# whwh747/A-Low-Texture-Robust-Hybrid-Feature-Based-Visual-Odometry

Measured on AMD Instinct MI355X. Metric: RGB-D frames/sec (640×480, 1k ORB + LSD + PEAC) at 1/2/4/8 GPUs, higher is better.
Workload: dtype u8/u16 integer + f32/f64; 1 GPU; 640x480 synthetic RGB-D, 1000 ORB (quota; 3/4 std + 1/4 lowtex scenes) + LSD lines + PEAC planes, 8192 frames per GPU per step (std640); frames_per_gpu=8192, parallelism=frames sharded, 1 rank(s), no data-path collective, distinct_frames=256, resident_bytes_per_frame_estimate=21100000

## Files before the change

a-low-texture-robust-hybrid-feature-based-visual-odometry_amd/__init__.py:

```python
import ctypes as C
import os
import subprocess
import numpy as np

_HERE = os.path.dirname(os.path.abspath(__file__))
_CSRC = os.path.join(_HERE, "csrc")
_LIBPATH = os.environ.get("HVO_LIB") or os.path.join(_CSRC, "libhvo.so")
_LIB = None
_LOADED_BEFORE_TORCH = False

HVO_OK = 0
STAGE_ORB, STAGE_LSD, STAGE_PLANES, STAGE_ALL = 1, 2, 4, 7
SLAB_LABELS = 1
STAGE_LSD_CULL = 8
STAGE_LINES3D, STAGE_VP, STAGE_PLANE_TAIL, STAGE_GRIDS = 16, 32, 64, 128
STAGE_FRAME = 1 | 2 | 8 | 4 | 16 | 32 | 64 | 128
LINE_MATCH_NNR, LINE_MATCH_BF, LINE_MATCH_DOUBLE = 0, 1, 2

KEYPOINT_DT = np.dtype([("x", "<f4"), ("y", "<f4"), ("size", "<f4"), ("angle", "<f4"),
                        ("response", "<f4"), ("octave", "<i4"), ("class_id", "<i4")])
KEYLINE_DT = np.dtype([("angle", "<f4"), ("class_id", "<i4"), ("octave", "<i4"),
                       ("pt_x", "<f4"), ("pt_y", "<f4"), ("response", "<f4"), ("size", "<f4"),
                       ("sx", "<f4"), ("sy", "<f4"), ("ex", "<f4"), ("ey", "<f4"),
                       ("sox", "<f4"), ("soy", "<f4"), ("eox", "<f4"), ("eoy", "<f4"),
# ... 1123 lines not shown
        self._chk(lib().hvo_normals_lpvo(self.h, _p(depth), w, h, depth.strides[0], _p(nrm), _p(dz), _p(px), cap, C.byref(n)), "normals_lpvo")
        return nrm[: n.value], dz[: n.value], px[: n.value]

    def surface_normals(self, depth):
        depth = np.ascontiguousarray(depth, np.uint16); h, w = depth.shape
        cap = (((h + 2) // 3) // 2) * (((w + 2) // 3) // 2)
        out = np.zeros(max(cap, 1), SURFACE_NORMAL_DT); n = C.c_int(0)
        self._chk(lib().hvo_surface_normals(self.h, _p(depth), w, h, depth.strides[0], _p(out), cap, C.byref(n)), "surface_normals")
        return out[: n.value].copy()

    def lsd_images(self, frame=0):
        L = lib()
        L.hvo_debug_lsd_images.argtypes = [C.c_void_p, C.c_int, C.POINTER(C.c_int), C.POINTER(C.c_int), C.c_void_p, C.c_void_p, C.c_longlong, C.POINTER(C.c_longlong), C.c_void_p]
        L.hvo_debug_lsd_images.restype = C.c_int
        w, h = self._w, self._h
        sw, sh = int(round(w * 0.8)), int(round(h * 0.8))
        mask = np.zeros((sh, (sw + 31) // 32), np.uint32); rec = np.zeros((sw * sh, 4), np.float64); dxy = np.zeros((h, w, 2), np.int16)
        n = C.c_longlong(0); csw = C.c_int(0); csh = C.c_int(0)
        self._chk(L.hvo_debug_lsd_images(self.h, frame, C.byref(csw), C.byref(csh), _p(mask), _p(rec), len(rec), C.byref(n), _p(dxy)), "lsd_images")
        if (csw.value, csh.value) != (sw, sh):
            raise HvoError(-1, "lsd_images: the plan's scaled size is %d x %d" % (csw.value, csh.value))
        return {"mask": mask, "records": rec[:n.value].copy(), "dxy": dxy}

    def peac_stats(self, frame=0):
        L = lib()
        L.hvo_debug_peac_stats.argtypes = [C.c_void_p, C.c_int, C.c_void_p]; L.hvo_debug_peac_stats.restype = C.c_int
        m = np.zeros(16, np.int32)
        self._chk(L.hvo_debug_peac_stats(self.h, frame, _p(m)), "peac_stats")
        return {"segments": int(m[0]), "coarse_planes": int(m[2]), "flags": int(m[3]), "planes": int(m[4]), "queue_entries": int(m[5]),
                "flood_rounds": int(m[8]), "flood_ranked_rounds": int(m[9]), "flood_serial_rounds": int(m[10]), "ahc_rounds": int(m[11]), "ahc_stops_no_head": int(m[12]), "ahc_stops_conflict": int(m[13]), "ahc_stops_key_order": int(m[14])}

    def hamming_matrix(self, q, t):
        q = np.ascontiguousarray(q, np.uint8).reshape(-1, 32); t = np.ascontiguousarray(t, np.uint8).reshape(-1, 32)
        d = np.zeros((len(q), len(t)), np.uint16)
        self._chk(lib().hvo_hamming_matrix(self.h, _p(q), len(q), _p(t), len(t), _p(d)), "hamming_matrix")
        return d

    def hamming_knn2(self, q, t):
        q = np.ascontiguousarray(q, np.uint8).reshape(-1, 32); t = np.ascontiguousarray(t, np.uint8).reshape(-1, 32)
        idx = np.zeros((len(q), 2), np.int32); dist = np.zeros((len(q), 2), np.int32)
        self._chk(lib().hvo_hamming_knn2(self.h, _p(q), len(q), _p(t), len(t), _p(idx), _p(dist)), "hamming_knn2")
        return idx, dist

    def match_nnr(self, d1, d2, nnr):
        d1 = np.ascontiguousarray(d1, np.uint8).reshape(-1, 32); d2 = np.ascontiguousarray(d2, np.uint8).reshape(-1, 32)
        m = np.full(len(d1), -1, np.int32); n = C.c_int(0)
# ... 869 lines not shown
```

a-low-texture-robust-hybrid-feature-based-visual-odometry_amd/csrc/lsd.hip:

```cpp
#include "hvo_internal.hpp"
#include <math.h>
#include <string.h>
#include <vector>
#include <algorithm>

#define LSD_PI 3.1415926535897932384626433832795
#define LSD_NOTDEF (-1024.0)
#ifndef LSD_RING
#define LSD_RING 256
#endif

static double lsd_sqrt_threshold(double rho)
{
    double c = rho * rho;
    while (sqrt(nextafter(c, INFINITY)) <= rho) c = nextafter(c, INFINITY);
    while (sqrt(c) > rho) c = nextafter(c, 0.0);
    return c;
}

struct LsdPlan {
    int w = 0, h = 0, sw = 0, sh = 0, batch = 0, nfeat = 0, nwords = 0;
    double *d_blur = nullptr;
    int chunk = 0;
    double4 *d_px = nullptr;
    bool compact = false; double4 *d_pool = nullptr; size_t pool_cap = 0;
    unsigned *d_defmask = nullptr, *d_wprefix = nullptr;
    long long *d_fbase = nullptr; int *d_fcount = nullptr; unsigned long long *d_pooltop = nullptr;
    unsigned *d_defined = nullptr;
    int *d_reg = nullptr;
    float *d_segs = nullptr;
    hvo_keyline *d_kl_all = nullptr;
    int maxseg = 0;
    hvo_keyline *d_kl = nullptr; uint8_t *d_desc = nullptr; double *d_fn = nullptr; int *d_nkl = nullptr; int *d_flags = nullptr;
    hvo_keyline *d_kl2 = nullptr; uint8_t *d_desc2 = nullptr; double *d_fn2 = nullptr; int *d_nkl2 = nullptr;
    uint8_t *d_b5 = nullptr; short2 *d_dxy = nullptr;
    int *d_xofs = nullptr, *d_yofs = nullptr; float *d_xa = nullptr, *d_yb = nullptr;
    double k7[4] = { 0, 0, 0, 0 };
    int k5[3] = { 0, 0, 0 };
    double gL[21], gG[63];
    float *d_gL = nullptr, *d_gG = nullptr;
    double rho = 0, prec = 0, p = 0; unsigned min_reg = 0;
    double rhoT = 0;
    long long *d_stats = nullptr;
    bool pre_fused = true;
    struct { Knob dense, lat, async_w, async_early, async_lds, lat_lds, lbd_split, spin_max; } kn;
    uint8_t *d_b8 = nullptr, *d_s8 = nullptr; int *d_rs8tab = nullptr;
    size_t async_w_cap = 0;
    int *d_redo = nullptr; int async_last_n = 0, async_last_w = 0;
    int async_b = 0; unsigned *d_atags = nullptr; void *d_actl = nullptr; int *d_alists = nullptr, *d_ablk = nullptr, *d_afreg = nullptr; unsigned char *d_ainreg = nullptr; int ainreg_b = 0;
};
static LsdPlan *plan_of(hvo_ctx *ctx) { return (LsdPlan *)ctx->lsd; }

static __device__ __forceinline__ int refl(int p, int n) { if (p < 0) p = -p; if (p >= n) p = 2 * (n - 1) - p; return p < 0 ? 0 : p; }

static __device__ __forceinline__ float fatan2_deg(float y, float x)
{
    const float p1 = 0.9997878412794807f * (float)(180 / 3.14159265358979323846);
    const float p3 = -0.3258083974640975f * (float)(180 / 3.14159265358979323846);
    const float p5 = 0.1555786518463281f * (float)(180 / 3.14159265358979323846);
    const float p7 = -0.04432655554792128f * (float)(180 / 3.14159265358979323846);
    const float eps = (float)2.2204460492503131e-16;
    const float ax = fabsf(x), ay = fabsf(y);
    const bool hi = ax >= ay;
    const float c = __fdiv_rn(hi ? ay : ax, __fadd_rn(hi ? ax : ay, eps)), c2 = __fmul_rn(c, c);
    float r = __fmul_rn(__fadd_rn(__fmul_rn(__fadd_rn(__fmul_rn(__fadd_rn(__fmul_rn(p7, c2), p5), c2), p3), c2), p1), c);
    if (!hi) r = __fsub_rn(90.f, r);
    if (x < 0) r = __fsub_rn(180.f, r);
    if (y < 0) r = __fsub_rn(360.f, r);
// ... 1021 lines not shown
        rowstep(v + 1, nB, nA);
    }
    if (v == v1) rowstep(v, nA, nB);
    if (yb + LBD_FUSED_ROWS >= h) store_edge(h - 1, nA, nB);
}

template <bool AL>
__global__ __launch_bounds__(256) void k_lbd_blur_sobel(const uint8_t *__restrict__ gray, size_t gframe, int gpitch,
                                                        short2 *__restrict__ dxy, int w, int h, int k0, int k1, int k2)
{
    const int nstrip = (w + 3) >> 2, item = blockIdx.x * 256 + threadIdx.x, f = blockIdx.z;
    const int rb = item / nstrip;
    const int x0 = (item - rb * nstrip) * 4, yb = rb * LBD_FUSED_ROWS;
    if (yb >= h) return;
    lbd_blur_sobel_body<AL>(gray + (size_t)f * gframe, gpitch, dxy + (size_t)f * h * w, w, h, x0, yb, k0, k1, k2);
}

__constant__ int c_lbd_comb[32][2] = {
    { 0, 1 }, { 0, 2 }, { 0, 3 }, { 0, 4 }, { 0, 5 }, { 0, 6 }, { 1, 2 }, { 1, 3 }, { 1, 4 }, { 1, 5 }, { 1, 6 },
    { 2, 3 }, { 2, 4 }, { 2, 5 }, { 2, 6 }, { 2, 7 }, { 2, 8 }, { 3, 4 }, { 3, 5 }, { 3, 6 }, { 3, 7 }, { 3, 8 },
    { 4, 5 }, { 4, 6 }, { 4, 7 }, { 4, 8 }, { 5, 6 }, { 5, 7 }, { 5, 8 }, { 6, 7 }, { 6, 8 }, { 7, 8 } };

#define LBD_UNR 8
__global__ __launch_bounds__(64) void k_lbd_desc(const short2 *__restrict__ dxyImg, int w, int h,
                                                 const hvo_keyline *__restrict__ kls, const int *__restrict__ nkl, int kl_cap,
                                                 const float *__restrict__ gL, const float *__restrict__ gG, uint8_t *__restrict__ desc)
{
    __shared__ float rows[63][4];
    __shared__ float band[9][8];
    __shared__ float dv[72];
    const int line = blockIdx.x, f = blockIdx.y, t = threadIdx.x;
    if (line >= nkl[f]) return;
    const hvo_keyline kl = kls[(size_t)f * kl_cap + line];
    const short2 *DXY = dxyImg + (size_t)f * w * h;
    const short imageWidth = (short)(w - 1), imageHeight = (short)(h - 1);
    const short halfHeight = 31;
    const short lengthOfLSP = (short)kl.num_pixels;
    const short halfWidth = (short)((lengthOfLSP - 1) / 2);
    const float midX = (float)(0.5 * (double)__fadd_rn(kl.sox, kl.eox));
    const float midY = (float)(0.5 * (double)__fadd_rn(kl.soy, kl.eoy));
    const float dL0 = (float)cos((double)kl.angle), dL1 = (float)sin((double)kl.angle);
    const float dO0 = -dL1, dO1 = dL0;
    __shared__ int tile[63 * 33];
    const bool along_rows = fabsf(dL0) > fabsf(dL1);
    float sCorX = 0, sCorY = 0, pL = 0, nL = 0, pO = 0, nO = 0;
    if (t < 63) {
        float sCorX0 = __fadd_rn(__fadd_rn(__fmul_rn(-dL0, (float)halfWidth), __fmul_rn(dL1, (float)halfHeight)), midX);
        float sCorY0 = __fadd_rn(__fsub_rn(__fmul_rn(-dL1, (float)halfWidth), __fmul_rn(dL0, (float)halfHeight)), midY);
        for (int q = 0; q < t; q++) { sCorX0 = __fsub_rn(sCorX0, dL1); sCorY0 = __fadd_rn(sCorY0, dL0); }
// ... 107 lines not shown
        }
        tempM = __fdiv_rn(1.f, sqrtf(tempM)); tempS = __fdiv_rn(1.f, sqrtf(tempS));
        v0 = __fmul_rn(v0, (t & 7) < 4 ? tempM : tempS); v1 = __fmul_rn(v1, (t & 7) < 4 ? tempM : tempS);
        if ((double)v0 > 0.4) v0 = (float)0.4;
        if ((double)v1 > 0.4) v1 = (float)0.4;
        p0 = __fmul_rn(v0, v0); p1 = __fmul_rn(v1, v1);
        float tmp = 0;
#pragma unroll
        for (int i = 0; i < 72; i++) tmp = __fadd_rn(tmp, i < 64 ? lane_of(p0, i & 63) : lane_of(p1, i & 7));
        tmp = __fdiv_rn(1.f, sqrtf(tmp));
        __syncthreads();
        dv[t] = __fmul_rn(v0, tmp);
        if (t < 8) dv[64 + t] = __fmul_rn(v1, tmp);
    }
    __syncthreads();
    if (t < 32) {
        const float *f1 = dv + 8 * c_lbd_comb[t][0], *f2 = dv + 8 * c_lbd_comb[t][1];
        unsigned r = 0;
        for (int b = 0; b < 8; b++) if (f1[b] > f2[b]) r |= 1u << b;
        desc[((size_t)f * kl_cap + line) * 32 + t] = (uint8_t)r;
    }
}


#define CULL_MAXL 2048
struct CullArgs {
    const hvo_keyline *kl; const double *fn; const int *nkl; hvo_keyline *tmp; hvo_keyline *kl_out; double *fn_out; int *nkl_out;
    int cap, tmp_stride, w, h; double dis, cos_th, endpoint_dis;
};

static __device__ double cull_point_line_distance(const float *l, float px, float py)
{
    const double x0 = (double)px, y0 = (double)py, x1 = l[0], y1 = l[1], x2 = l[2], y2 = l[3];
    return fabs((y2 - y1) * x0 + (x1 - x2) * y0 + ((x2 * y1) - (x1 * y2))) / sqrt((y2 - y1) * (y2 - y1) + (x1 - x2) * (x1 - x2));
}
static __device__ double cull_two_line_angle(const double *f1, const double *f2)
{
    double v1[3] = { f1[0], f1[1], f1[2] }, v2[3] = { f2[0], f2[1], f2[2] };
    v1[0] /= v1[2]; v1[1] /= v1[2];
    v2[0] /= v2[2]; v2[1] /= v2[2];
    const double a0 = v1[0] / v1[2], a1 = v1[1] / v1[2], b0 = v2[0] / v2[2], b1 = v2[1] / v2[2];
    const double a = a0 * b0 + a1 * b1;
    const double b = sqrt(a0 * a0 + a1 * a1), c = sqrt(b0 * b0 + b1 * b1);
    return fabs(a / (b * c));
}
static __device__ void cull_merge_two_lines(const float *l1, const float *l2, float *out)
// ... 110 lines not shown
    double *fo = a.fn_out + (size_t)f * a.cap * 3;
    for (int i = lane; i < m; i += 64) {
        const float r = resp[i];
        int rank = 0;
        for (int q = 0; q < m; q++) { const float rq = resp[q]; rank += (rq > r) || (rq == r && q < i); }
        hvo_keyline k = tmp[i]; k.class_id = rank;
        if (rank < a.cap) {
            out[rank] = k;
            const double sx = k.sx, sy = k.sy, ex = k.ex, ey = k.ey;
            const double l0 = sy * 1.0 - 1.0 * ey, l1 = 1.0 * ex - sx * 1.0, l2 = sx * ey - sy * ex;
            const double nrm = sqrt(l0 * l0 + l1 * l1);
            fo[3 * rank] = l0 / nrm; fo[3 * rank + 1] = l1 / nrm; fo[3 * rank + 2] = l2 / nrm;
        }
    }
    if (lane == 0) a.nkl_out[f] = m;
}

void lsd_free(hvo_ctx *ctx)
{
    LsdPlan *P = plan_of(ctx);
    if (!P) return;
    void *ptrs[] = { P->d_kl2, P->d_desc2, P->d_fn2, P->d_nkl2, P->d_blur, P->d_px, P->d_defined, P->d_reg, P->d_segs, P->d_kl_all, P->d_kl,
                     P->d_desc, P->d_fn, P->d_nkl, P->d_flags, P->d_b5, P->d_dxy, P->d_xofs, P->d_yofs, P->d_xa, P->d_yb, P->d_gL, P->d_gG, P->d_stats,
                     P->d_pool, P->d_defmask, P->d_wprefix, P->d_fbase, P->d_fcount, P->d_pooltop, P->d_atags, P->d_actl, P->d_alists, P->d_ablk, P->d_afreg, P->d_ainreg, P->d_redo, P->d_b8, P->d_s8, P->d_rs8tab };
    for (void *q : ptrs) if (q) (void)hipFree(q);
    delete P;
    ctx->lsd = nullptr;
}

static int cvfloor_f(float v) { int i = (int)v; return i - (i > v); }

static int lsd_build_plan(hvo_ctx *ctx, int w, int h, int batch);
static int lsd_ensure_plan(hvo_ctx *ctx, int w, int h, int batch)
{
    LsdPlan *P = plan_of(ctx);
    if (P && P->w == w && P->h == h && P->batch >= batch) return HVO_OK;
    lsd_free(ctx);
    const int rc = lsd_build_plan(ctx, w, h, batch);
    if (rc) lsd_free(ctx);
    return rc;
}

static int lsd_build_plan(hvo_ctx *ctx, int w, int h, int batch)
{
    LsdPlan *P = new LsdPlan();
    ctx->lsd = P;
    P->w = w; P->h = h; P->batch = batch; P->nfeat = std::max(ctx->p.lsd_nfeatures, 1);
// ... 22 lines not shown
        for (int i = 0; i < 21; i++) { double d = i - u; P->gL[i] = exp(d * d * inv); }
        u = (9 * 7 - 1) / 2; sigma = u; inv = -1 / (2 * sigma * sigma);
        for (int i = 0; i < 63; i++) { double d = i - u; P->gG[i] = exp(d * d * inv); }
    }
    std::vector<int> xofs(P->sw), yofs(P->sh + PRE_CH, 0); std::vector<float> xa(2 * P->sw), yb(2 * (P->sh + PRE_CH), 0.f);
    const double scale = 1. / SCALE;
    for (int dx = 0; dx < P->sw; dx++) {
        float fx = (float)((dx + 0.5) * scale - 0.5); int sx = cvfloor_f(fx); fx -= sx;
        if (sx < 0) { fx = 0; sx = 0; }
        if (sx >= w - 1) { fx = 0; sx = w - 1; }
        xofs[dx] = sx; xa[2 * dx] = 1.f - fx; xa[2 * dx + 1] = fx;
    }
    for (int dy = 0; dy < P->sh; dy++) {
        float fy = (float)((dy + 0.5) * scale - 0.5); int sy = cvfloor_f(fy); fy -= sy;
        int sy0 = std::min(std::max(sy, 0), h - 1), sy1 = std::min(std::max(sy + 1, 0), h - 1);
        yofs[dy] = sy0 | (sy1 << 16); yb[2 * dy] = 1.f - fy; yb[2 * dy + 1] = fy;
    }
    std::vector<float> gLf(21), gGf(63);
    for (int i = 0; i < 21; i++) gLf[i] = (float)P->gL[i];
    for (int i = 0; i < 63; i++) gGf[i] = (float)P->gG[i];
    const size_t B = batch, npix = (size_t)w * h, nsp = (size_t)P->sw * P->sh;
#define PA(ptr, n) HVO_HIP(hipMalloc((void **)&(ptr), (n)))
    P->kn.dense.read("HVO_LSD_DENSE"); P->kn.lat.read("HVO_LSD_LAT"); P->kn.async_w.read("HVO_LSD_ASYNC"); P->kn.async_early.read("HVO_LSD_ASYNC_EARLY");
    P->kn.async_lds.read("HVO_LSD_ASYNC_LDS"); P->kn.lat_lds.read("HVO_LSD_LAT_LDS"); P->kn.lbd_split.read("HVO_LBD_SPLIT"); P->kn.spin_max.read("HVO_LSD_ASYNC_SPIN_MAX");
    P->chunk = (int)std::min<size_t>(B, 512);
    { const char *e = getenv("HVO_LSD_CHUNK"); if (e && atoi(e) > 0) P->chunk = (int)std::min<size_t>(B, (size_t)atoi(e)); }
    P->compact = false;
    { const char *e = getenv("HVO_LSD_COMPACT"); if (e) P->compact = atoi(e) != 0; }
    double frac = 0.27;
    { const char *e = getenv("HVO_LSD_COMPACT_FRAC"); if (e && atof(e) > 0) frac = std::min(1.0, atof(e)); }
    if (P->compact) {
        const size_t fit = std::max<size_t>(64, (size_t)(3.3e9 / (double)(nsp * sizeof(double4))) / 64 * 64);
        P->chunk = (int)std::min<size_t>((size_t)P->chunk, std::min<size_t>(fit, 512));
    }
    const size_t CB = (size_t)P->chunk;
    { const char *e = getenv("HVO_LSD_PRE_SPLIT"); P->pre_fused = !(e && atoi(e) != 0); }
    if (!P->pre_fused) PA(P->d_blur, CB * npix * 8);
    if (P->compact) {
        PA(P->d_px, CB * nsp * sizeof(double4));
        P->pool_cap = std::max<size_t>((size_t)((double)(B * nsp) * frac), 4096);
        PA(P->d_pool, P->pool_cap * sizeof(double4));
        PA(P->d_defmask, B * P->nwords * 4); PA(P->d_wprefix, B * P->nwords * 4);
        PA(P->d_fbase, B * 8); PA(P->d_fcount, B * 4); PA(P->d_pooltop, 16);
    } else
        PA(P->d_px, B * nsp * sizeof(double4));
    PA(P->d_defined, B * P->nwords * 4); PA(P->d_reg, B * nsp * 4);
    PA(P->d_segs, B * P->maxseg * 16); PA(P->d_kl_all, B * P->maxseg * sizeof(hvo_keyline));
    PA(P->d_kl, B * P->nfeat * sizeof(hvo_keyline)); PA(P->d_desc, B * P->nfeat * 32); PA(P->d_fn, B * P->nfeat * 24);
    PA(P->d_nkl, B * 4); PA(P->d_flags, B * 4);
    PA(P->d_kl2, B * P->nfeat * sizeof(hvo_keyline)); PA(P->d_desc2, B * P->nfeat * 32); PA(P->d_fn2, B * P->nfeat * 24); PA(P->d_nkl2, B * 4);
    if (P->kn.lbd_split.set) PA(P->d_b5, CB * npix);
    PA(P->d_dxy, CB * npix * sizeof(short2));
    PA(P->d_xofs, P->sw * 4); PA(P->d_yofs, (P->sh + PRE_CH) * 4); PA(P->d_xa, P->sw * 8); PA(P->d_yb, (P->sh + PRE_CH) * 8);
    PA(P->d_gL, 21 * 4); PA(P->d_gG, 63 * 4); PA(P->d_stats, B * 64);
    if (P->pre_fused) {
        int maxc = 0;
        for (int x0 = 0; x0 < P->sw; x0 += PRE_TW) { const int xe = std::min(x0 + PRE_TW, P->sw - 1); maxc = std::max(maxc, std::min(xofs[xe] + 1, w - 1) - xofs[x0] + 1); }
        int maxr = 0;
        for (int ys = 0; ys < P->sh; ys += PRE_CH) maxr = std::max(maxr, (yofs[std::min(ys + PRE_CH - 1, P->sh - 1)] >> 16) - (yofs[ys] & 0xFFFF) + 1);
        if (maxc > 256 || maxr > PRE_RING) { P->pre_fused = false; PA(P->d_blur, CB * npix * 8); }
    }
#undef PA
    HVO_HIP(hipMemcpy(P->d_xofs, xofs.data(), P->sw * 4, hipMemcpyHostToDevice));
    HVO_HIP(hipMemcpy(P->d_yofs, yofs.data(), yofs.size() * 4, hipMemcpyHostToDevice));
    HVO_HIP(hipMemcpy(P->d_xa, xa.data(), P->sw * 8, hipMemcpyHostToDevice));
    HVO_HIP(hipMemcpy(P->d_yb, yb.data(), yb.size() * 4, hipMemcpyHostToDevice));
    HVO_HIP(hipMemcpy(P->d_gL, gLf.data(), 21 * 4, hipMemcpyHostToDevice));
    HVO_HIP(hipMemcpy(P->d_gG, gGf.data(), 63 * 4, hipMemcpyHostToDevice));
    HVO_HIP(hipMemsetAsync(P->d_defined, 0, B * P->nwords * 4, ctx->s_lsd));
    HVO_HIP(hipMemsetAsync(P->d_nkl, 0, B * 4, ctx->s_lsd));
    HVO_HIP(hipMemsetAsync(P->d_nkl2, 0, B * 4, ctx->s_lsd));
    HVO_HIP(hipMemsetAsync(P->d_flags, 0, B * 4, ctx->s_lsd));
    HVO_HIP(hipDeviceSynchronize());
    return HVO_OK;
}

int lsd_prepare(hvo_ctx *ctx, int w, int h, int batch, bool culled, LsdView *v)
{
    int rc = lsd_ensure_plan(ctx, w, h, batch);
    if (rc) return rc;
    LsdPlan *P = plan_of(ctx);
    v->d_kl = culled ? P->d_kl2 : P->d_kl; v->d_desc = culled ? P->d_desc2 : P->d_desc; v->d_fn = culled ? P->d_fn2 : P->d_fn;
    v->d_nkl = culled ? P->d_nkl2 : P->d_nkl; v->d_flags = P->d_flags; v->nfeat = P->nfeat;
    return HVO_OK;
}

int lsd_run(hvo_ctx *ctx, int n, bool cull)
{
    OrbPlan &O = ctx->orb;
    if (O.w <= 0 || n < 1 || n > O.batch) return HVO_ERR_INVALID_ARG;
    int rc = lsd_ensure_plan(ctx, O.w, O.h, std::max(n, ctx->p.max_batch));
    if (rc) return rc;
    LsdPlan *P = plan_of(ctx);
    P->async_last_n = P->async_last_w = 0;
    hipStream_t st = hvo_stream_lsd(ctx);
    const int w = P->w, h = P->h, sw = P->sw, sh = P->sh;
    const uint8_t *gray = O.d_pyr + O.lev[0].img_off;
    const int gpitch = O.lev[0].pitch;
    int id;
    const size_t nsp = (size_t)sw * sh;
    const int gx = (((sw + 31) & ~31) + 255) / 256;
    for (int attempt = 0; attempt < 3; attempt++) {
        if (P->compact) HVO_HIP(hipMemsetAsync(P->d_pooltop, 0, 16, st));
        for (int c0 = 0; c0 < n; c0 += P->chunk) {
            const int m = std::min(P->chunk, n - c0);
            if (ctx->readings & HVO_READING_LSD_8U) {
                id = hvo_prof_begin(ctx, "lsd_gradient", st);
// ... 93 lines not shown
                                   P->d_px, P->d_defined, P->nwords, P->rho);
            { GrowArgs g2 = g; g2.redo = 1; g2.redo_count = P->d_redo; g2.perm = nullptr; hipLaunchKernelGGL(k_lsd_grow, dim3(n), dim3(64), 0, st, g2); }
        }
    } else aw = 0;
    if (aw > 0) {
    } else if (lat) {
        size_t lds = (size_t)P->nwords * 4, floor_ = 56 * 1024;
        if (P->kn.lat_lds.set) floor_ = (size_t)std::max(P->kn.lat_lds.v, 0);
        if (lds < floor_ && floor_ <= 150 * 1024) lds = floor_;
        if (hvo_ensure_dyn_lds(reinterpret_cast<const void *>(k_lsd_grow_lat), lds)) return HVO_ERR_HIP;
        hipLaunchKernelGGL(k_lsd_grow_lat, dim3(n), dim3(64), lds, st, g);
    } else if (P->compact) {
        if (dense) hipLaunchKernelGGL(k_lsd_grow_dense_c, dim3(n), dim3(64), 0, st, g);
        else hipLaunchKernelGGL(k_lsd_grow_c, dim3(n), dim3(64), 0, st, g);
    } else if (dense) hipLaunchKernelGGL(k_lsd_grow_dense, dim3(n), dim3(64), 0, st, g);
    else hipLaunchKernelGGL(k_lsd_grow, dim3(n), dim3(64), 0, st, g);
    hvo_prof_end(ctx, id);
    if (cull && P->nfeat > CULL_MAXL) return HVO_ERR_UNSUPPORTED;
    for (int c0 = 0; c0 < n; c0 += P->chunk) {
        const int m = std::min(P->chunk, n - c0);
        const uint8_t *gc = gray + (size_t)c0 * O.pyr_bytes;
        const size_t ko = (size_t)c0 * P->nfeat;
        id = hvo_prof_begin(ctx, "lbd_sobel", st);
        if (ctx->readings & HVO_READING_BLUR_FLOAT) {
            if (!P->d_b5) HVO_HIP(hipMalloc((void **)&P->d_b5, (size_t)P->chunk * w * h));
            if ((rc = readings_gblur_enqueue(st, gc, O.pyr_bytes, gpitch, w, h, P->d_b5, (size_t)w * h, w, m, 5, 1.0, true))) return rc;
            hipLaunchKernelGGL(k_lbd_sobel, dim3((w + 255) / 256, (h + LBD_BLUR_ROWS - 1) / LBD_BLUR_ROWS, m), dim3(256), 0, st, P->d_b5, P->d_dxy, w, h);
        } else
        if (P->d_b5) {
            hipLaunchKernelGGL(k_lbd_blur5, dim3((w + 255) / 256, (h + LBD_BLUR_ROWS - 1) / LBD_BLUR_ROWS, m), dim3(256), 0, st, gc, O.pyr_bytes, gpitch, P->d_b5, w, h, P->k5[0], P->k5[1], P->k5[2]);
            hipLaunchKernelGGL(k_lbd_sobel, dim3((w + 255) / 256, (h + LBD_BLUR_ROWS - 1) / LBD_BLUR_ROWS, m), dim3(256), 0, st, P->d_b5, P->d_dxy, w, h);
        } else
{
            const dim3 grid((((w + 3) / 4) * ((h + LBD_FUSED_ROWS - 1) / LBD_FUSED_ROWS) + 255) / 256, 1, m);
            if ((w & 3) == 0) hipLaunchKernelGGL(k_lbd_blur_sobel<true>, grid, dim3(256), 0, st, gc, O.pyr_bytes, gpitch, P->d_dxy, w, h, P->k5[0], P->k5[1], P->k5[2]);
            else hipLaunchKernelGGL(k_lbd_blur_sobel<false>, grid, dim3(256), 0, st, gc, O.pyr_bytes, gpitch, P->d_dxy, w, h, P->k5[0], P->k5[1], P->k5[2]);
        }
        hvo_prof_end(ctx, id);
        id = hvo_prof_begin(ctx, "lbd_desc", st);
        hipLaunchKernelGGL(k_lbd_desc, dim3(P->nfeat, m), dim3(64), 0, st, P->d_dxy, w, h, P->d_kl + ko, P->d_nkl + c0, P->nfeat, P->d_gL, P->d_gG, P->d_desc + ko * 32);
        hvo_prof_end(ctx, id);
        if (cull) {
            id = hvo_prof_begin(ctx, "lsd_cull", st);
            CullArgs c;
            c.kl = P->d_kl + ko; c.fn = P->d_fn + ko * 3; c.nkl = P->d_nkl + c0; c.tmp = P->d_kl_all + (size_t)c0 * P->maxseg; c.tmp_stride = P->maxseg;
            c.kl_out = P->d_kl2 + ko; c.fn_out = P->d_fn2 + ko * 3; c.nkl_out = P->d_nkl2 + c0;
            c.cap = P->nfeat; c.w = w; c.h = h; c.dis = ctx->cull_dis; c.cos_th = cos(ctx->cull_angle * 0.0174533); c.endpoint_dis = ctx->cull_endpoint;
            const int maxl = (P->nfeat + 63) & ~63;
            if (hvo_ensure_dyn_lds(reinterpret_cast<const void *>(k_cull_lines), cull_lds_bytes(maxl))) return HVO_ERR_HIP;
            hipLaunchKernelGGL(k_cull_lines, dim3(m), dim3(64), cull_lds_bytes(maxl), st, c, maxl);
            hipLaunchKernelGGL(k_lbd_desc, dim3(P->nfeat, m), dim3(64), 0, st, P->d_dxy, w, h, P->d_kl2 + ko, P->d_nkl2 + c0, P->nfeat, P->d_gL, P->d_gG, P->d_desc2 + ko * 32);
            hvo_prof_end(ctx, id);
        }
    }
    HVO_HIP(hipGetLastError());
    return HVO_OK;
}

int lsd_download(hvo_ctx *ctx, int n, hvo_frame_out *out, bool culled)
{
    const hipStream_t cs = hvo_copy_stream(ctx, ctx->s_lsd);
    LsdPlan *P = plan_of(ctx);
    if (!P) return HVO_ERR_INVALID_ARG;
    const hvo_keyline *d_kl = culled ? P->d_kl2 : P->d_kl; const uint8_t *d_desc = culled ? P->d_desc2 : P->d_desc;
    const double *d_fn = culled ? P->d_fn2 : P->d_fn; const int *d_nkl = culled ? P->d_nkl2 : P->d_nkl;
    std::vector<int> nk(n), fl(n);
    HVO_HIP(hipMemcpyAsync(nk.data(), d_nkl, n * sizeof(int), hipMemcpyDeviceToHost, cs));
    HVO_HIP(hipMemcpyAsync(fl.data(), P->d_flags, n * sizeof(int), hipMemcpyDeviceToHost, cs));
    HVO_HIP(hipStreamSynchronize(cs));
    std::vector<void *> d0(n, nullptr), d1(n, nullptr), d2(n, nullptr); std::vector<size_t> b0(n, 0), b1(n, 0), b2(n, 0);
    for (int f = 0; f < n; f++) {
        int m = nk[f];
        if (fl[f]) out[f].status = HVO_ERR_CAPACITY;
        if (out[f].kl) {
// ... 125 lines not shown
                           P->d_xofs, P->d_xa, P->d_yofs, P->d_yb, px, def, P->nwords, P->rho);
    }
    HVO_HIP(hipGetLastError());
    HVO_HIP(hipStreamSynchronize(st));
    HVO_HIP(hipMemcpy(mask, def, (size_t)P->nwords * 4, hipMemcpyDeviceToHost));
    std::vector<double> rec2(nsp * 4);
    HVO_HIP(hipMemcpy(rec2.data(), px, nsp * sizeof(double4), hipMemcpyDeviceToHost));
    const int wpr = (sw + 31) / 32;
    long long n = 0;
    for (int y = 0; y < sh; y++)
        for (int x = 0; x < sw; x++) {
            if (!((mask[(size_t)y * wpr + (x >> 5)] >> (x & 31)) & 1u)) continue;
            const size_t i = ((size_t)y * sw + x) * 4;
            if (memcmp(&rec[i], &rec2[i], 32) != 0) { ctx->last_error = "lsd images: a record of the run differs from the one formed again"; return HVO_ERR_HIP; }
            if (n < rec_cap) memcpy(records + n * 4, &rec[i], 32);
            n++;
        }
    *n_records = n;
    if (sw_out) *sw_out = sw;
    if (sh_out) *sh_out = sh;
    return HVO_OK;
}

extern "C" int hvo_lsd_async_report(hvo_ctx *ctx, int *frames_regrown, int *foreign_workers, int *workers_per_frame)
{
    LsdPlan *P = ctx ? plan_of(ctx) : nullptr;
    if (!ctx) return HVO_ERR_INVALID_ARG;
    if (frames_regrown) *frames_regrown = 0;
    if (foreign_workers) *foreign_workers = 0;
    if (workers_per_frame) *workers_per_frame = 0;
    if (!P || !P->d_actl || P->async_last_n < 1) return HVO_OK;
    if (hipSetDevice(ctx->device) != hipSuccess) return HVO_ERR_NO_DEVICE;
    HVO_HIP(hipStreamSynchronize(hvo_stream_lsd(ctx)));
    int redo = 0;
    HVO_HIP(hipMemcpy(&redo, P->d_redo, 4, hipMemcpyDeviceToHost));
    std::vector<LaCtl> ctl((size_t)P->async_last_n);
    HVO_HIP(hipMemcpy(ctl.data(), P->d_actl, ctl.size() * sizeof(LaCtl), hipMemcpyDeviceToHost));
    int nf = 0;
    for (const LaCtl &c : ctl) nf += (int)c.n_foreign;
    if (frames_regrown) *frames_regrown = redo;
    if (foreign_workers) *foreign_workers = nf;
    if (workers_per_frame) *workers_per_frame = P->async_last_w;
    return HVO_OK;
}

extern "C" int hvo_debug_lsd_async(hvo_ctx *ctx, int frame, unsigned *out64)
// ... 7 lines not shown
```

Before: 58740 frames/s.

## Rework LBD descriptor with precomputed line rows and LDS-staged gradient gathers

Adds a setup kernel that precomputes each keyline's 63 row start points, direction and length into a scratch buffer. The new LBD descriptor kernel reads these records, and for mostly-horizontal lines stages sample addresses in shared memory. Threads then transpose so the gradient gathers run across the line rather than across rows, giving better coalescing. It also treats short2 gradients as packed ints with cheaper clamp and rounding. The cost is an extra launch and a scratch buffer of about 512 bytes per line. The old kernel stays available via HVO_LBD_DESC=off, and a debug entry point is added.

Result: faster. 60050 frames/s, median of 6 (+2.2%).

```diff
diff --git a/a-low-texture-robust-hybrid-feature-based-visual-odometry_amd/__init__.py b/a-low-texture-robust-hybrid-feature-based-visual-odometry_amd/__init__.py
--- a/a-low-texture-robust-hybrid-feature-based-visual-odometry_amd/__init__.py
+++ b/a-low-texture-robust-hybrid-feature-based-visual-odometry_amd/__init__.py
@@ -1169,6 +1169,16 @@
             raise HvoError(-1, "lsd_images: the plan's scaled size is %d x %d" % (csw.value, csh.value))
         return {"mask": mask, "records": rec[:n.value].copy(), "dxy": dxy}
 
+    def lbd_desc(self, gray, keylines):
+        L = lib()
+        L.hvo_debug_lbd_desc.argtypes = [C.c_void_p, C.c_void_p, C.c_int, C.c_int, C.c_int, C.c_void_p, C.c_int, C.c_void_p]
+        L.hvo_debug_lbd_desc.restype = C.c_int
+        gray = np.ascontiguousarray(gray, np.uint8); h, w = gray.shape
+        kl = np.ascontiguousarray(keylines, KEYLINE_DT)
+        desc = np.zeros((len(kl), 32), np.uint8)
+        self._chk(L.hvo_debug_lbd_desc(self.h, _p(gray), w, h, gray.strides[0], _p(kl), len(kl), _p(desc)), "lbd_desc")
+        return desc
+
     def peac_stats(self, frame=0):
         L = lib()
         L.hvo_debug_peac_stats.argtypes = [C.c_void_p, C.c_int, C.c_void_p]; L.hvo_debug_peac_stats.restype = C.c_int
diff --git a/a-low-texture-robust-hybrid-feature-based-visual-odometry_amd/csrc/lsd.hip b/a-low-texture-robust-hybrid-feature-based-visual-odometry_amd/csrc/lsd.hip
--- a/a-low-texture-robust-hybrid-feature-based-visual-odometry_amd/csrc/lsd.hip
+++ b/a-low-texture-robust-hybrid-feature-based-visual-odometry_amd/csrc/lsd.hip
@@ -34,6 +34,7 @@
     hvo_keyline *d_kl = nullptr; uint8_t *d_desc = nullptr; double *d_fn = nullptr; int *d_nkl = nullptr; int *d_flags = nullptr;
     hvo_keyline *d_kl2 = nullptr; uint8_t *d_desc2 = nullptr; double *d_fn2 = nullptr; int *d_nkl2 = nullptr;
     uint8_t *d_b5 = nullptr; short2 *d_dxy = nullptr;
+    struct LbdLine *d_lbdl = nullptr;
     int *d_xofs = nullptr, *d_yofs = nullptr; float *d_xa = nullptr, *d_yb = nullptr;
     double k7[4] = { 0, 0, 0, 0 };
     int k5[3] = { 0, 0, 0 };
@@ -43,7 +44,7 @@
     double rhoT = 0;
     long long *d_stats = nullptr;
     bool pre_fused = true;
-    struct { Knob dense, lat, async_w, async_early, async_lds, lat_lds, lbd_split, spin_max; } kn;
+    struct { Knob dense, lat, async_w, async_early, async_lds, lat_lds, lbd_split, lbd_desc, spin_max; } kn;
     uint8_t *d_b8 = nullptr, *d_s8 = nullptr; int *d_rs8tab = nullptr;
     size_t async_w_cap = 0;
     int *d_redo = nullptr; int async_last_n = 0, async_last_w = 0;
@@ -1111,9 +1112,9 @@
     { 4, 5 }, { 4, 6 }, { 4, 7 }, { 4, 8 }, { 5, 6 }, { 5, 7 }, { 5, 8 }, { 6, 7 }, { 6, 8 }, { 7, 8 } };
 
 #define LBD_UNR 8
-__global__ __launch_bounds__(64) void k_lbd_desc(const short2 *__restrict__ dxyImg, int w, int h,
-                                                 const hvo_keyline *__restrict__ kls, const int *__restrict__ nkl, int kl_cap,
-                                                 const float *__restrict__ gL, const float *__restrict__ gG, uint8_t *__restrict__ desc)
+__global__ __launch_bounds__(64) void k_lbd_desc_v1(const short2 *__restrict__ dxyImg, int w, int h,
+                                                    const hvo_keyline *__restrict__ kls, const int *__restrict__ nkl, int kl_cap,
+                                                    const float *__restrict__ gL, const float *__restrict__ gG, uint8_t *__restrict__ desc)
 {
     __shared__ float rows[63][4];
     __shared__ float band[9][8];
@@ -1267,6 +1268,205 @@
     }
 }
 
+#define LBD_SHORT_SAFE 16000
+struct LbdLine { float2 row[63]; float dL0, dL1; int len, pad; };
+
+__global__ __launch_bounds__(64) void k_lbd_line_setup(const hvo_keyline *__restrict__ kls, const int *__restrict__ nkl, int kl_cap, int nframes,
+                                                       LbdLine *__restrict__ out)
+{
+    const int i = blockIdx.x * 64 + threadIdx.x;
+    if (i >= nframes * kl_cap) return;
+    const int f = i / kl_cap;
+    if (i - f * kl_cap >= nkl[f]) return;
+    const hvo_keyline kl = kls[i];
+    const short halfHeight = 31;
+    const short lengthOfLSP = (short)kl.num_pixels;
+    const short halfWidth = (short)((lengthOfLSP - 1) / 2);
+    const float midX = (float)(0.5 * (double)__fadd_rn(kl.sox, kl.eox));
+    const float midY = (float)(0.5 * (double)__fadd_rn(kl.soy, kl.eoy));
+    const float dL0 = (float)cos((double)kl.angle), dL1 = (float)sin((double)kl.angle);
+    float sCorX0 = __fadd_rn(__fadd_rn(__fmul_rn(-dL0, (float)halfWidth), __fmul_rn(dL1, (float)halfHeight)), midX);
+    float sCorY0 = __fadd_rn(__fsub_rn(__fmul_rn(-dL1, (float)halfWidth), __fmul_rn(dL0, (float)halfHeight)), midY);
+    LbdLine *o = out + i;
+    o->row[0] = make_float2(sCorX0, sCorY0);
+    for (int q = 1; q < 63; q++) {
+        sCorX0 = __fsub_rn(sCorX0, dL1); sCorY0 = __fadd_rn(sCorY0, dL0);
+        o->row[q] = make_float2(sCorX0, sCorY0);
+    }
+    o->dL0 = dL0; o->dL1 = dL1; o->len = (int)lengthOfLSP; o->pad = 0;
+}
+
+static __device__ __forceinline__ unsigned lbd_round_clamp(float x, float hi)
+{
+    return (unsigned)__builtin_amdgcn_fmed3f(__fadd_rn(x, copysignf(0x1.fffffep-2f, x)), 0.f, hi);
+}
+template <int N> struct LbdN { static constexpr int value = N; };
+
+__global__ __launch_bounds__(64) void k_lbd_desc(const int *__restrict__ dxyImg, int w, int h,
+                                                 const LbdLine *__restrict__ lines, const int *__restrict__ nkl, int kl_cap,
+                                                 const float *__restrict__ gL, const float *__restrict__ gG, uint8_t *__restrict__ desc)
+{
+    __shared__ __align__(16) int tile[64 * 33];
+    float (*rows)[4] = reinterpret_cast<float (*)[4]>(tile);
+    float *band = reinterpret_cast<float *>(tile) + 320;
+    float *sqMS = reinterpret_cast<float *>(tile) + 400;
+    float *sqAll = reinterpret_cast<float *>(tile) + 480;
+    float *dv = reinterpret_cast<float *>(tile) + 560;
+    const int line = blockIdx.x, f = blockIdx.y, t = threadIdx.x;
+    if (line >= nkl[f]) return;
+    const LbdLine *L = lines + ((size_t)f * kl_cap + line);
+    const float dL0 = L->dL0, dL1 = L->dL1;
+    const int len = max(L->len, 0);
+    const char *DXY = reinterpret_cast<const char *>(dxyImg + (size_t)f * w * h);
+    const float xmax = (float)(w - 1), ymax = (float)(h - 1);
+    const unsigned pitch = 4u * (unsigned)w;
+    auto sample = [&](unsigned a) { return *reinterpret_cast<const int *>(DXY + a); };
+    const float2 start = L->row[min(t, 62)];
+    float sCorX = start.x, sCorY = start.y, pL = 0, nL = 0, pO = 0, nO = 0;
+    auto next_addr = [&]() {
+        const unsigned xCor = lbd_round_clamp(sCorX, xmax), yCor = lbd_round_clamp(sCorY, ymax);
+        sCorX = __fadd_rn(sCorX, dL0); sCorY = __fadd_rn(sCorY, dL1);
+        return __umul24(yCor, pitch) + (xCor << 2);
+    };
+    auto accumulate = [&](int g) {
+        const float ddx = (float)(short)(g & 0xFFFF), ddy = (float)(g >> 16);
+        const float gDL = __fadd_rn(__fmul_rn(ddx, dL0), __fmul_rn(ddy, dL1));
+        const float gDO = __fadd_rn(__fmul_rn(ddx, -dL1), __fmul_rn(ddy, dL0));
+        pL = __fadd_rn(pL, fmaxf(gDL, 0.f)); nL = __fsub_rn(nL, fminf(gDL, 0.f));
+        pO = __fadd_rn(pO, fmaxf(gDO, 0.f)); nO = __fsub_rn(nO, fminf(gDO, 0.f));
+    };
+    if (fabsf(dL0) > fabsf(dL1)) {
+        int *mine = tile + t * 33;
+        auto fill = [&](auto n, int u0) {
+#pragma unroll
+            for (int u = 0; u < decltype(n)::value; u++) mine[u0 + u] = (int)next_addr();
+        };
+        auto take = [&](auto n, int u0) {
+#pragma unroll
+            for (int u = 0; u < decltype(n)::value; u++) accumulate(mine[u0 + u]);
+        };
+        for (int w0 = 0; w0 < len; w0 += 32) {
+            const int nu = min(32, len - w0);
+            if (nu == 32) { for (int u0 = 0; u0 < 32; u0 += 8) fill(LbdN<8>(), u0); }
+            else {
+                int u0 = 0;
+                if (nu & 16) { fill(LbdN<16>(), u0); u0 += 16; }
+                if (nu & 8) { fill(LbdN<8>(), u0); u0 += 8; }
+                if (nu & 4) { fill(LbdN<4>(), u0); u0 += 4; }
+                if (nu & 2) { fill(LbdN<2>(), u0); u0 += 2; }
+                if (nu & 1) fill(LbdN<1>(), u0);
+            }
+            __syncthreads();
+            {
+                const int u = t & 31, rh = t >> 5;
+                if (u < nu) {
+                    for (int r0 = 0; r0 < 64; r0 += 16) {
+                        int av[8], gv[8];
+#pragma unroll
+                        for (int k = 0; k < 8; k++) av[k] = tile[(r0 + 2 * k + rh) * 33 + u];
+#pragma unroll
+                        for (int k = 0; k < 8; k++) gv[k] = sample((unsigned)av[k]);
+#pragma unroll
+                        for (int k = 0; k < 8; k++) tile[(r0 + 2 * k + rh) * 33 + u] = gv[k];
+                    }
+                }
+            }
+            __syncthreads();
+            if (nu == 32) { for (int u0 = 0; u0 < 32; u0 += 8) take(LbdN<8>(), u0); }
+            else {
+                int u0 = 0;
+                if (nu & 16) { take(LbdN<16>(), u0); u0 += 16; }
+                if (nu & 8) { take(LbdN<8>(), u0); u0 += 8; }
+                if (nu & 4) { take(LbdN<4>(), u0); u0 += 4; }
+                if (nu & 2) { take(LbdN<2>(), u0); u0 += 2; }
+                if (nu & 1) take(LbdN<1>(), u0);
+            }
+            __syncthreads();
+        }
+    } else {
+        auto block = [&](auto n) {
+            int g[decltype(n)::value];
+#pragma unroll
+            for (int u = 0; u < decltype(n)::value; u++) g[u] = sample(next_addr());
+#pragma unroll
+            for (int u = 0; u < decltype(n)::value; u++) accumulate(g[u]);
+        };
+        int w0 = 0;
+        for (; w0 + LBD_UNR <= len; w0 += LBD_UNR) block(LbdN<LBD_UNR>());
+        const int nu = len - w0;
+        if (nu & 4) block(LbdN<4>());
+        if (nu & 2) block(LbdN<2>());
+        if (nu & 1) block(LbdN<1>());
+    }
+    if (t < 28) { reinterpret_cast<float *>(tile)[t] = 0.f; reinterpret_cast<float *>(tile)[70 * 4 + t] = 0.f; }
+    if (t < 63) {
+        const float coef = gG[t];
+        *reinterpret_cast<float4 *>(rows[7 + t]) = make_float4(__fmul_rn(coef, pL), __fmul_rn(coef, nL), __fmul_rn(coef, pO), __fmul_rn(coef, nO));
+    }
+    __syncthreads();
+    {
+        const int q = t & 7;
+        const bool sq = (q & 2) != 0;
+        const float *r0 = &rows[7 * (t >> 3)][(q & 1) + 2 * (q >> 2)], *r1 = &rows[56][(q & 1) + 2 * (q >> 2)];
+        float s0 = 0, s1 = 0;
+#pragma unroll
+        for (int j = 0; j < 21; j++) {
+            const float c = gL[j], cc = __fmul_rn(c, c);
+            const float k = sq ? cc : c;
+            const float a0 = r0[4 * j], a1 = r1[4 * j];
+            s0 = __fadd_rn(s0, __fmul_rn(k, sq ? __fmul_rn(a0, a0) : a0));
+            s1 = __fadd_rn(s1, __fmul_rn(k, sq ? __fmul_rn(a1, a1) : a1));
+        }
+        band[t] = s0;
+        if (t < 8) band[64 + t] = s1;
+    }
+    __syncthreads();
+    float v0, v1;
+    {
+        const int o = t & 7, qm = (o & 1) | ((o & 2) << 1);
+        auto value = [&](int b) {
+            const float invN = (b == 0 || b == 8) ? (float)(1.0 / 14.0) : (float)(1.0 / 21.0);
+            const float tmp = __fmul_rn(band[8 * b + qm], invN);
+            const float dev = sqrtf(__fsub_rn(__fmul_rn(band[8 * b + qm + 2], invN), __fmul_rn(tmp, tmp)));
+            return o < 4 ? tmp : dev;
+        };
+        v0 = value(t >> 3); v1 = value(8);
+        float *dst = sqMS + 36 * (o >> 2) + (o & 3);
+        dst[4 * (t >> 3)] = __fmul_rn(v0, v0);
+        if (t < 8) dst[32] = __fmul_rn(v1, v1);
+    }
+    __syncthreads();
+    auto ordered_sum = [](const float *p, int n4) {
+        float s = 0;
+        for (int i = 0; i < n4; i++) {
+            const float4 x = reinterpret_cast<const float4 *>(p)[i];
+            s = __fadd_rn(__fadd_rn(__fadd_rn(__fadd_rn(s, x.x), x.y), x.z), x.w);
+        }
+        return s;
+    };
+    {
+        const float scale = __fdiv_rn(1.f, sqrtf(ordered_sum(sqMS + 36 * ((t & 7) >> 2), 9)));
+        v0 = __fmul_rn(v0, scale); v1 = __fmul_rn(v1, scale);
+        if ((double)v0 > 0.4) v0 = (float)0.4;
+        if ((double)v1 > 0.4) v1 = (float)0.4;
+        sqAll[t] = __fmul_rn(v0, v0);
+        if (t < 8) sqAll[64 + t] = __fmul_rn(v1, v1);
+    }
+    __syncthreads();
+    {
+        const float tmp = __fdiv_rn(1.f, sqrtf(ordered_sum(sqAll, 18)));
+        dv[t] = __fmul_rn(v0, tmp);
+        if (t < 8) dv[64 + t] = __fmul_rn(v1, tmp);
+    }
+    __syncthreads();
+    if (t < 32) {
+        const float *f1 = dv + 8 * c_lbd_comb[t][0], *f2 = dv + 8 * c_lbd_comb[t][1];
+        unsigned r = 0;
+        for (int b = 0; b < 8; b++) if (f1[b] > f2[b]) r |= 1u << b;
+        desc[((size_t)f * kl_cap + line) * 32 + t] = (uint8_t)r;
+    }
+}
+
 
 #define CULL_MAXL 2048
 struct CullArgs {
@@ -1423,7 +1623,7 @@
     if (!P) return;
     void *ptrs[] = { P->d_kl2, P->d_desc2, P->d_fn2, P->d_nkl2, P->d_blur, P->d_px, P->d_defined, P->d_reg, P->d_segs, P->d_kl_all, P->d_kl,
                      P->d_desc, P->d_fn, P->d_nkl, P->d_flags, P->d_b5, P->d_dxy, P->d_xofs, P->d_yofs, P->d_xa, P->d_yb, P->d_gL, P->d_gG, P->d_stats,
-                     P->d_pool, P->d_defmask, P->d_wprefix, P->d_fbase, P->d_fcount, P->d_pooltop, P->d_atags, P->d_actl, P->d_alists, P->d_ablk, P->d_afreg, P->d_ainreg, P->d_redo, P->d_b8, P->d_s8, P->d_rs8tab };
+                     P->d_pool, P->d_defmask, P->d_wprefix, P->d_fbase, P->d_fcount, P->d_pooltop, P->d_atags, P->d_actl, P->d_alists, P->d_ablk, P->d_afreg, P->d_ainreg, P->d_redo, P->d_b8, P->d_s8, P->d_rs8tab, P->d_lbdl };
     for (void *q : ptrs) if (q) (void)hipFree(q);
     delete P;
     ctx->lsd = nullptr;
@@ -1492,7 +1692,7 @@
     const size_t B = batch, npix = (size_t)w * h, nsp = (size_t)P->sw * P->sh;
 #define PA(ptr, n) HVO_HIP(hipMalloc((void **)&(ptr), (n)))
     P->kn.dense.read("HVO_LSD_DENSE"); P->kn.lat.read("HVO_LSD_LAT"); P->kn.async_w.read("HVO_LSD_ASYNC"); P->kn.async_early.read("HVO_LSD_ASYNC_EARLY");
-    P->kn.async_lds.read("HVO_LSD_ASYNC_LDS"); P->kn.lat_lds.read("HVO_LSD_LAT_LDS"); P->kn.lbd_split.read("HVO_LBD_SPLIT"); P->kn.spin_max.read("HVO_LSD_ASYNC_SPIN_MAX");
+    P->kn.async_lds.read("HVO_LSD_ASYNC_LDS"); P->kn.lat_lds.read("HVO_LSD_LAT_LDS"); P->kn.lbd_split.read("HVO_LBD_SPLIT"); P->kn.lbd_desc.read("HVO_LBD_DESC"); P->kn.spin_max.read("HVO_LSD_ASYNC_SPIN_MAX");
     P->chunk = (int)std::min<size_t>(B, 512);
     { const char *e = getenv("HVO_LSD_CHUNK"); if (e && atoi(e) > 0) P->chunk = (int)std::min<size_t>(B, (size_t)atoi(e)); }
     P->compact = false;
@@ -1521,6 +1721,7 @@
     PA(P->d_kl2, B * P->nfeat * sizeof(hvo_keyline)); PA(P->d_desc2, B * P->nfeat * 32); PA(P->d_fn2, B * P->nfeat * 24); PA(P->d_nkl2, B * 4);
     if (P->kn.lbd_split.set) PA(P->d_b5, CB * npix);
     PA(P->d_dxy, CB * npix * sizeof(short2));
+    if (!P->kn.lbd_desc.off() && std::max(w, h) <= LBD_SHORT_SAFE) PA(P->d_lbdl, CB * P->nfeat * sizeof(LbdLine));
     PA(P->d_xofs, P->sw * 4); PA(P->d_yofs, (P->sh + PRE_CH) * 4); PA(P->d_xa, P->sw * 8); PA(P->d_yb, (P->sh + PRE_CH) * 8);
     PA(P->d_gL, 21 * 4); PA(P->d_gG, 63 * 4); PA(P->d_stats, B * 64);
     if (P->pre_fused) {
@@ -1553,6 +1754,36 @@
     v->d_kl = culled ? P->d_kl2 : P->d_kl; v->d_desc = culled ? P->d_desc2 : P->d_desc; v->d_fn = culled ? P->d_fn2 : P->d_fn;
     v->d_nkl = culled ? P->d_nkl2 : P->d_nkl; v->d_flags = P->d_flags; v->nfeat = P->nfeat;
     return HVO_OK;
+}
+
+static int lbd_sobel_enqueue(hvo_ctx *ctx, LsdPlan *P, hipStream_t st, const uint8_t *gc, int m)
+{
+    OrbPlan &O = ctx->orb;
+    const int w = P->w, h = P->h, gpitch = O.lev[0].pitch;
+    int rc;
+    if (ctx->readings & HVO_READING_BLUR_FLOAT) {
+        if (!P->d_b5) HVO_HIP(hipMalloc((void **)&P->d_b5, (size_t)P->chunk * w * h));
+        if ((rc = readings_gblur_enqueue(st, gc, O.pyr_bytes, gpitch, w, h, P->d_b5, (size_t)w * h, w, m, 5, 1.0, true))) return rc;
+        hipLaunchKernelGGL(k_lbd_sobel, dim3((w + 255) / 256, (h + LBD_BLUR_ROWS - 1) / LBD_BLUR_ROWS, m), dim3(256), 0, st, P->d_b5, P->d_dxy, w, h);
+    } else if (P->d_b5) {
+        hipLaunchKernelGGL(k_lbd_blur5, dim3((w + 255) / 256, (h + LBD_BLUR_ROWS - 1) / LBD_BLUR_ROWS, m), dim3(256), 0, st, gc, O.pyr_bytes, gpitch, P->d_b5, w, h, P->k5[0], P->k5[1], P->k5[2]);
+        hipLaunchKernelGGL(k_lbd_sobel, dim3((w + 255) / 256, (h + LBD_BLUR_ROWS - 1) / LBD_BLUR_ROWS, m), dim3(256), 0, st, P->d_b5, P->d_dxy, w, h);
+    } else {
+        const dim3 grid((((w + 3) / 4) * ((h + LBD_FUSED_ROWS - 1) / LBD_FUSED_ROWS) + 255) / 256, 1, m);
+        if ((w & 3) == 0) hipLaunchKernelGGL(k_lbd_blur_sobel<true>, grid, dim3(256), 0, st, gc, O.pyr_bytes, gpitch, P->d_dxy, w, h, P->k5[0], P->k5[1], P->k5[2]);
+        else hipLaunchKernelGGL(k_lbd_blur_sobel<false>, grid, dim3(256), 0, st, gc, O.pyr_bytes, gpitch, P->d_dxy, w, h, P->k5[0], P->k5[1], P->k5[2]);
+    }
+    return HVO_OK;
+}
+
+static void lbd_desc_enqueue(const LsdPlan *P, hipStream_t st, int m, const hvo_keyline *kl, const int *nkl, int kl_cap, LbdLine *scratch, uint8_t *desc)
+{
+    if (!scratch) {
+        hipLaunchKernelGGL(k_lbd_desc_v1, dim3(kl_cap, m), dim3(64), 0, st, P->d_dxy, P->w, P->h, kl, nkl, kl_cap, P->d_gL, P->d_gG, desc);
+        return;
+    }
+    hipLaunchKernelGGL(k_lbd_line_setup, dim3((unsigned)(((size_t)kl_cap * m + 63) / 64)), dim3(64), 0, st, kl, nkl, kl_cap, m, scratch);
+    hipLaunchKernelGGL(k_lbd_desc, dim3(kl_cap, m), dim3(64), 0, st, reinterpret_cast<const int *>(P->d_dxy), P->w, P->h, (const LbdLine *)scratch, nkl, kl_cap, P->d_gL, P->d_gG, desc);
 }
 
 int lsd_run(hvo_ctx *ctx, int n, bool cull)
@@ -1692,23 +1923,10 @@
         const uint8_t *gc = gray + (size_t)c0 * O.pyr_bytes;
         const size_t ko = (size_t)c0 * P->nfeat;
         id = hvo_prof_begin(ctx, "lbd_sobel", st);
-        if (ctx->readings & HVO_READING_BLUR_FLOAT) {
-            if (!P->d_b5) HVO_HIP(hipMalloc((void **)&P->d_b5, (size_t)P->chunk * w * h));
-            if ((rc = readings_gblur_enqueue(st, gc, O.pyr_bytes, gpitch, w, h, P->d_b5, (size_t)w * h, w, m, 5, 1.0, true))) return rc;
-            hipLaunchKernelGGL(k_lbd_sobel, dim3((w + 255) / 256, (h + LBD_BLUR_ROWS - 1) / LBD_BLUR_ROWS, m), dim3(256), 0, st, P->d_b5, P->d_dxy, w, h);
-        } else
-        if (P->d_b5) {
-            hipLaunchKernelGGL(k_lbd_blur5, dim3((w + 255) / 256, (h + LBD_BLUR_ROWS - 1) / LBD_BLUR_ROWS, m), dim3(256), 0, st, gc, O.pyr_bytes, gpitch, P->d_b5, w, h, P->k5[0], P->k5[1], P->k5[2]);
-            hipLaunchKernelGGL(k_lbd_sobel, dim3((w + 255) / 256, (h + LBD_BLUR_ROWS - 1) / LBD_BLUR_ROWS, m), dim3(256), 0, st, P->d_b5, P->d_dxy, w, h);
-        } else
-{
-            const dim3 grid((((w + 3) / 4) * ((h + LBD_FUSED_ROWS - 1) / LBD_FUSED_ROWS) + 255) / 256, 1, m);
-            if ((w & 3) == 0) hipLaunchKernelGGL(k_lbd_blur_sobel<true>, grid, dim3(256), 0, st, gc, O.pyr_bytes, gpitch, P->d_dxy, w, h, P->k5[0], P->k5[1], P->k5[2]);
-            else hipLaunchKernelGGL(k_lbd_blur_sobel<false>, grid, dim3(256), 0, st, gc, O.pyr_bytes, gpitch, P->d_dxy, w, h, P->k5[0], P->k5[1], P->k5[2]);
-        }
+        if ((rc = lbd_sobel_enqueue(ctx, P, st, gc, m))) return rc;
         hvo_prof_end(ctx, id);
         id = hvo_prof_begin(ctx, "lbd_desc", st);
-        hipLaunchKernelGGL(k_lbd_desc, dim3(P->nfeat, m), dim3(64), 0, st, P->d_dxy, w, h, P->d_kl + ko, P->d_nkl + c0, P->nfeat, P->d_gL, P->d_gG, P->d_desc + ko * 32);
+        lbd_desc_enqueue(P, st, m, P->d_kl + ko, P->d_nkl + c0, P->nfeat, P->d_lbdl, P->d_desc + ko * 32);
         hvo_prof_end(ctx, id);
         if (cull) {
             id = hvo_prof_begin(ctx, "lsd_cull", st);
@@ -1719,7 +1937,7 @@
             const int maxl = (P->nfeat + 63) & ~63;
             if (hvo_ensure_dyn_lds(reinterpret_cast<const void *>(k_cull_lines), cull_lds_bytes(maxl))) return HVO_ERR_HIP;
             hipLaunchKernelGGL(k_cull_lines, dim3(m), dim3(64), cull_lds_bytes(maxl), st, c, maxl);
-            hipLaunchKernelGGL(k_lbd_desc, dim3(P->nfeat, m), dim3(64), 0, st, P->d_dxy, w, h, P->d_kl2 + ko, P->d_nkl2 + c0, P->nfeat, P->d_gL, P->d_gG, P->d_desc2 + ko * 32);
+            lbd_desc_enqueue(P, st, m, P->d_kl2 + ko, P->d_nkl2 + c0, P->nfeat, P->d_lbdl, P->d_desc2 + ko * 32);
             hvo_prof_end(ctx, id);
         }
     }
@@ -1891,6 +2109,41 @@
     return HVO_OK;
 }
 
+extern "C" int hvo_debug_lbd_desc(hvo_ctx *ctx, const uint8_t *gray, int w, int h, int stride, const hvo_keyline *keylines, int n, uint8_t *desc_out)
+{
+    if (!ctx || !gray || !keylines || !desc_out || w <= 0 || h <= 0 || stride < w || n < 1 || n > (1 << 20)) return HVO_ERR_INVALID_ARG;
+    for (int i = 0; i < n; i++) {
+        const hvo_keyline &k = keylines[i];
+        const float reach = 0.5f * (float)k.num_pixels + 32.f, mx = 0.5f * (k.sox + k.eox), my = 0.5f * (k.soy + k.eoy);
+        if (k.num_pixels < 0 || k.num_pixels > 32767 || !(fabsf(mx) + reach < 32000.f) || !(fabsf(my) + reach < 32000.f) || !(fabsf(k.angle) < 1e6f)) {
+            ctx->last_error = "lbd desc: a key line's samples would leave the range of a short"; return HVO_ERR_INVALID_ARG;
+        }
+    }
+    if (hipSetDevice(ctx->device) != hipSuccess) return HVO_ERR_NO_DEVICE;
+    hvo_frame_in in; memset(&in, 0, sizeof(in));
+    in.gray = gray; in.gray_stride = stride;
+    int rc = orb_upload(ctx, 1, &in, w, h);
+    if (rc) return rc;
+    ctx->last_stages = 0;
+    OrbPlan &O = ctx->orb;
+    if ((rc = lsd_ensure_plan(ctx, O.w, O.h, std::max(1, ctx->p.max_batch)))) return rc;
+    LsdPlan *P = plan_of(ctx);
+    hipStream_t st = hvo_stream_lsd(ctx);
+    hvo_keyline *d_kl = nullptr; int *d_n = nullptr; uint8_t *d_desc = nullptr; LbdLine *d_rec = nullptr;
+    bool ok = hipMalloc((void **)&d_kl, (size_t)n * sizeof(hvo_keyline)) == hipSuccess && hipMalloc((void **)&d_n, 4) == hipSuccess &&
+              hipMalloc((void **)&d_desc, (size_t)n * 32) == hipSuccess && (!P->d_lbdl || hipMalloc((void **)&d_rec, (size_t)n * sizeof(LbdLine)) == hipSuccess);
+    ok = ok && hipMemcpy(d_kl, keylines, (size_t)n * sizeof(hvo_keyline), hipMemcpyHostToDevice) == hipSuccess && hipMemcpy(d_n, &n, 4, hipMemcpyHostToDevice) == hipSuccess;
+    if (ok) {
+        rc = lbd_sobel_enqueue(ctx, P, st, O.d_pyr + O.lev[0].img_off, 1);
+        if (!rc) {
+            lbd_desc_enqueue(P, st, 1, d_kl, d_n, n, d_rec, d_desc);
+            ok = hipGetLastError() == hipSuccess && hipStreamSynchronize(st) == hipSuccess && hipMemcpy(desc_out, d_desc, (size_t)n * 32, hipMemcpyDeviceToHost) == hipSuccess;
+        }
+    }
+    (void)hipFree(d_kl); (void)hipFree(d_n); (void)hipFree(d_desc); (void)hipFree(d_rec);
+    return rc ? rc : ok ? HVO_OK : HVO_ERR_HIP;
+}
+
 extern "C" int hvo_lsd_async_report(hvo_ctx *ctx, int *frames_regrown, int *foreign_workers, int *workers_per_frame)
 {
     LsdPlan *P = ctx ? plan_of(ctx) : nullptr;
```
